# avi2924/Speech-Intent-Recognizer

Measured on AMD Instinct MI355X. Metric: utterances/sec (16 kHz, 3 s clips), inference: HIP STFT+mel+CNN/BiGRU forward + argmax, higher is better.
Workload: dtype f32

## Files before the change

speech-intent-recognizer_amd/csrc/f16x3_kernels.h:

```cpp
#pragma once
#include "bf16x6_kernels.h"

constexpr int H3_BM = 160, H3_BN = 256, H3_BK = 32;
constexpr int H3_APLANE = H3_BM * 64, H3_BPLANE = H3_BN * 64;
constexpr int H3_BOFF = 2 * H3_APLANE;
constexpr int H3_STAGE = H3_BOFF + 2 * H3_BPLANE;
constexpr int H3_APIECES = 2 * H3_BM / 16, H3_PIECES = H3_APIECES + 2 * H3_BN / 16;
constexpr int H3_PPW = (H3_PIECES + 7) / 8;
constexpr int h3_lds_bytes(int nst) { return nst * H3_STAGE; }

template <int BM>
struct H3Geo {
    static_assert(BM == 96 || BM == 128 || BM == 160, "BM = 96, 128 or 160");
    static constexpr int FR = BM / 32, ARG = BM / 16;
    static constexpr int APLANE = BM * 64, BOFF = 2 * APLANE, STAGE = BOFF + 2 * H3_BPLANE;
    static constexpr int APIECES = 2 * ARG, PIECES = APIECES + 2 * H3_BN / 16;
    static constexpr int PPW = (PIECES + 7) / 8, PREM = PIECES & 7;
    static constexpr int ISTRIDE = 3 * FR / PPW;
};
static_assert(H3Geo<H3_BM>::STAGE == H3_STAGE && H3Geo<H3_BM>::PIECES == H3_PIECES && H3Geo<H3_BM>::PPW == H3_PPW, "160-row geometry");

template <int FR>
__device__ __forceinline__ void h3_read_step(unsigned aaddr, unsigned baddr, f16x8 (&ah)[FR], f16x8 (&al)[FR], f16x8& bh, f16x8& bl) {
    if constexpr (FR == 5) {
        asm volatile(
            "ds_read_b128 %0, %12\n\t"
            "ds_read_b128 %10, %13 offset:20480\n\t"
            "ds_read_b128 %5, %12 offset:10240\n\t"
            "ds_read_b128 %11, %13 offset:36864\n\t"
            "ds_read_b128 %1, %12 offset:2048\n\t"
            "ds_read_b128 %6, %12 offset:12288\n\t"
            "ds_read_b128 %2, %12 offset:4096\n\t"
            "ds_read_b128 %7, %12 offset:14336\n\t"
            "ds_read_b128 %3, %12 offset:6144\n\t"
            "ds_read_b128 %8, %12 offset:16384\n\t"
            "ds_read_b128 %4, %12 offset:8192\n\t"
            "ds_read_b128 %9, %12 offset:18432\n\t"
            "s_waitcnt lgkmcnt(0)"
            : "=&v"(ah[0]), "=&v"(ah[1]), "=&v"(ah[2]), "=&v"(ah[3]), "=&v"(ah[4]),
              "=&v"(al[0]), "=&v"(al[1]), "=&v"(al[2]), "=&v"(al[3]), "=&v"(al[4]), "=&v"(bh), "=&v"(bl)
            : "v"(aaddr), "v"(baddr)
            : "memory");
    } else if constexpr (FR == 4) {
        asm volatile(
            "ds_read_b128 %0, %10\n\t"
            "ds_read_b128 %8, %11 offset:16384\n\t"
            "ds_read_b128 %4, %10 offset:8192\n\t"
            "ds_read_b128 %9, %11 offset:32768\n\t"
            "ds_read_b128 %1, %10 offset:2048\n\t"
            "ds_read_b128 %5, %10 offset:10240\n\t"
            "ds_read_b128 %2, %10 offset:4096\n\t"
            "ds_read_b128 %6, %10 offset:12288\n\t"
            "ds_read_b128 %3, %10 offset:6144\n\t"
            "ds_read_b128 %7, %10 offset:14336\n\t"
            "s_waitcnt lgkmcnt(0)"
            : "=&v"(ah[0]), "=&v"(ah[1]), "=&v"(ah[2]), "=&v"(ah[3]),
              "=&v"(al[0]), "=&v"(al[1]), "=&v"(al[2]), "=&v"(al[3]), "=&v"(bh), "=&v"(bl)
            : "v"(aaddr), "v"(baddr)
            : "memory");
    } else {
        static_assert(FR == 3, "3, 4 or 5 fragments");
        asm volatile(
            "ds_read_b128 %0, %8\n\t"
            "ds_read_b128 %6, %9 offset:12288\n\t"
            "ds_read_b128 %3, %8 offset:6144\n\t"
            "ds_read_b128 %7, %9 offset:28672\n\t"
            "ds_read_b128 %1, %8 offset:2048\n\t"
            "ds_read_b128 %4, %8 offset:8192\n\t"
            "ds_read_b128 %2, %8 offset:4096\n\t"
            "ds_read_b128 %5, %8 offset:10240\n\t"
            "s_waitcnt lgkmcnt(0)"
            : "=&v"(ah[0]), "=&v"(ah[1]), "=&v"(ah[2]), "=&v"(al[0]), "=&v"(al[1]), "=&v"(al[2]), "=&v"(bh), "=&v"(bl)
            : "v"(aaddr), "v"(baddr)
            : "memory");
    }
}

template <int NST, int KNOCK, int BM, bool GATHER>
__device__ __forceinline__ void h3_gemm_tile(
    const unsigned short* __restrict__ Ap, const unsigned short* __restrict__ Bp0, const unsigned short* __restrict__ Bp1,
    const float* __restrict__ bias0, const float* __restrict__ bias1, float* __restrict__ C, int ldc, int M, int MA, int N, int K,
    int wgid, const int* __restrict__ rows, int* rtab) {
    static_assert(NST == 2 || NST == 3, "two or three stages");
    using G = H3Geo<BM>;
    constexpr int FR = G::FR, PPW = G::PPW;
    extern __shared__ __attribute__((aligned(1024))) unsigned char h3_smem[];
    const int nbd = N / H3_BN, nb = 2 * nbd;
    const int mblk = wgid / nb, nbk = wgid - mblk * nb, z = nbk / nbd;
    const int m0 = mblk * BM, n0 = (nbk - z * nbd) * H3_BN;
    const unsigned short* __restrict__ Bp = z ? Bp1 : Bp0;
    const float* __restrict__ bias = z ? bias1 : bias0;
    const int tid = threadIdx.x, lane = tid & 63, wv = __builtin_amdgcn_readfirstlane(tid >> 6), m = lane & 31, h = lane >> 5;
    const size_t planeA = (size_t)MA * K, planeB = (size_t)N * K;

    const int lr = lane >> 2;
    const int csrc = (lane & 3) ^ ((lr >> 2) & 3);
    constexpr int AI = (G::APIECES + 7) / 8;
    int arow[AI];
#pragma unroll
    for (int i = 0; i < AI; ++i) {
        const int g = wv + 8 * i < G::APIECES ? wv + 8 * i : 0;
        const int row = m0 + (g % G::ARG) * 16 + lr;
        arow[i] = row < M ? row : M - 1;
    }
    int orow = 0;
    if (GATHER) {
        const int ro = m0 + tid < M ? m0 + tid : M - 1;
        orow = rows[ro];
#pragma unroll
        for (int i = 0; i < AI; ++i) arow[i] = rows[arow[i]];
    }
    unsigned int poff[PPW];
#pragma unroll
    for (int i = 0; i < PPW; ++i) {
        const int g = wv + 8 * i;
        const int gb = g - G::APIECES, pl = (gb >> 4) & 1, rg = gb & 15;
        if (GATHER) {
            const unsigned pa = i < AI ? (unsigned)((g < G::APIECES ? g / G::ARG : 0) * planeA + (size_t)arow[i < AI ? i : 0] * K + csrc * 8) : 0u;
            const unsigned pb = (unsigned)(pl * planeB + (size_t)(n0 + rg * 16 + lr) * K + csrc * 8);
            poff[i] = g < G::APIECES ? pa : pb;
        } else if (g < G::APIECES) {
            poff[i] = (unsigned int)(g / G::ARG * planeA + (size_t)arow[i < AI ? i : 0] * K + csrc * 8);
        } else {
            poff[i] = (unsigned int)(pl * planeB + (size_t)(n0 + rg * 16 + lr) * K + csrc * 8);
        }
    }
    if (GATHER) rtab[tid] = orow;
    auto piece = [&](int i, int kt, int buf) {
        if (KNOCK & 1) return;
        const int g = wv + 8 * i;
        if (g < G::PIECES) {
            const unsigned short* src = (g < G::APIECES ? Ap : Bp) + poff[i] + (size_t)kt * H3_BK;
            __builtin_amdgcn_global_load_lds((sir_gptr_t)src, (sir_lptr_t)(h3_smem + buf * G::STAGE + g * 1024), 16, 0, 0);
        }
    };

    f32x16 acc0[FR], acc1[FR];
#pragma unroll
    for (int mt = 0; mt < FR; ++mt)
#pragma unroll
        for (int r = 0; r < 16; ++r) { acc0[mt][r] = 0.0f; acc1[mt][r] = 0.0f; }

    const unsigned sbase = (unsigned)(uintptr_t)h3_smem;
    unsigned fa[2], fb[2];
#pragma unroll
    for (int ks = 0; ks < 2; ++ks) {
        fa[ks] = sbase + m * 64 + ((((ks << 1) | h) ^ ((m >> 2) & 3)) << 4);
        fb[ks] = fa[ks] + wv * 2048;
    }
    const int nk = K / H3_BK;

    auto compute = [&](int buf, auto issue_c, int ktn, int bufn) {
        constexpr bool ISSUE = decltype(issue_c)::value;
        const unsigned so = (unsigned)(buf * G::STAGE);
#pragma unroll
        for (int ks = 0; ks < 2; ++ks) {
            f16x8 ah[FR], al[FR], bh, bl;
            h3_read_step<FR>(fa[ks] + so, fb[ks] + so, ah, al, bh, bl);
#pragma unroll
            for (int t = 0; t < 3; ++t)
#pragma unroll
                for (int mt = 0; mt < FR; ++mt) {
                    if (KNOCK & 4) {
                        acc0[mt][0] += (float)ah[mt][0] * (float)bh[0] + (float)al[mt][1] * (float)bl[1];
                    } else {
                        if (t == 0) acc1[mt] = __builtin_amdgcn_mfma_f32_32x32x16_f16(al[mt], bh, acc1[mt], 0, 0, 0);
                        if (t == 1) acc1[mt] = __builtin_amdgcn_mfma_f32_32x32x16_f16(ah[mt], bl, acc1[mt], 0, 0, 0);
                        if (t == 2) acc0[mt] = __builtin_amdgcn_mfma_f32_32x32x16_f16(ah[mt], bh, acc0[mt], 0, 0, 0);
                    }
                    const int idx = t * FR + mt;
                    if (ISSUE && idx % G::ISTRIDE == G::ISTRIDE - 1 && idx / G::ISTRIDE < PPW && ks == (wv >> 2))
                        piece(idx / G::ISTRIDE, ktn, bufn);
                }
            __builtin_amdgcn_sched_barrier(0);
        }
    };

#pragma unroll
    for (int s = 0; s < NST - 1; ++s)
        if (s < nk) {
#pragma unroll
            for (int i = 0; i < PPW; ++i) piece(i, s, s);
        }
    auto tile_wait = [&](bool more) {
        if (NST == 2 || !more) asm volatile("s_waitcnt vmcnt(0)" ::: "memory");
        else if (G::PREM == 0 || wv < G::PREM) asm volatile("s_waitcnt vmcnt(%0)" :: "n"(PPW) : "memory");
        else asm volatile("s_waitcnt vmcnt(%0)" :: "n"(PPW - 1) : "memory");
        asm volatile("s_barrier" ::: "memory");
    };
    int buf = 0, bufn = NST - 1, kt = 0;
    for (; kt + NST - 1 < nk; ++kt) {
        tile_wait(true);
        compute(buf, std::true_type{}, kt + NST - 1, bufn);
        buf = buf + 1 == NST ? 0 : buf + 1;
        bufn = bufn + 1 == NST ? 0 : bufn + 1;
    }
    for (; kt < nk; ++kt) {
        tile_wait(kt + 1 < nk);
        compute(buf, std::false_type{}, 0, 0);
        buf = buf + 1 == NST ? 0 : buf + 1;
    }

    const int n = n0 + wv * 32 + m;
    const float bv = bias ? bias[n] : 0.0f;
    if (GATHER) {
        float* cz = C + (size_t)z * N + n;
#pragma unroll
        for (int mt = 0; mt < FR; ++mt)
#pragma unroll
            for (int i = 0; i < 4; ++i) {
                const int4 g4 = *reinterpret_cast<const int4*>(rtab + mt * 32 + 8 * i + 4 * h);
                const int gr[4] = {g4.x, g4.y, g4.z, g4.w};
#pragma unroll
                for (int j = 0; j < 4; ++j) cz[gr[j] * ldc] = fmaf(acc1[mt][4 * i + j], H3_LO_INV, acc0[mt][4 * i + j]) + bv;
            }
        return;
    }
    float* crow = C + (size_t)(m0 + 4 * h) * ldc + (size_t)z * N + n;
    if (m0 + BM <= M) {
#pragma unroll
        for (int mt = 0; mt < FR; ++mt)
#pragma unroll
            for (int r = 0; r < 16; ++r)
                crow[(size_t)(mt * 32 + (r & 3) + 8 * (r >> 2)) * ldc] = fmaf(acc1[mt][r], H3_LO_INV, acc0[mt][r]) + bv;
    } else {
#pragma unroll
        for (int mt = 0; mt < FR; ++mt)
#pragma unroll
            for (int r = 0; r < 16; ++r) {
                const int ro = mt * 32 + (r & 3) + 8 * (r >> 2);
                if (m0 + 4 * h + ro < M) crow[(size_t)ro * ldc] = fmaf(acc1[mt][r], H3_LO_INV, acc0[mt][r]) + bv;
            }
    }
}

__device__ __forceinline__ int h3_xcd_tile(int orig, int nt) {
    const int xcd = orig & 7, q = nt >> 3, rem = nt & 7;
    return (xcd < rem ? xcd * (q + 1) : rem * (q + 1) + (xcd - rem) * q) + (orig >> 3);
}

template <int NST = 3, int KNOCK = 0>
static __global__ __launch_bounds__(512) void gemm_nt_f16x3_kernel(
    const unsigned short* __restrict__ Ap, const unsigned short* __restrict__ Bp0, const unsigned short* __restrict__ Bp1,
    const float* __restrict__ bias0, const float* __restrict__ bias1, float* __restrict__ C, int ldc, int M, int N, int K) {
    h3_gemm_tile<NST, KNOCK, H3_BM, false>(Ap, Bp0, Bp1, bias0, bias1, C, ldc, M, M, N, K, h3_xcd_tile(blockIdx.x, gridDim.x), nullptr, nullptr);
}

__host__ __device__ constexpr int h3_gather_tiles(int bm, int count, int N) { return (count + bm - 1) / bm * 2 * (N / H3_BN); }
__host__ __device__ constexpr int h3_gather_bm(int count, int N, int ncu) {
    return h3_gather_tiles(96, count, N) <= ncu ? 96 : h3_gather_tiles(128, count, N) <= ncu ? 128 : 160;
}
__host__ __device__ constexpr int h3_gather_cost(int bm, int K) {
    return K > 512 ? (bm == 96 ? 402 : bm == 128 ? 447 : 513) : (bm == 96 ? 236 : bm == 128 ? 261 : 294);
}
constexpr int H3_TP_FLOOR = 108;
__host__ __device__ constexpr int h3_gather_bm_throughput(int count, int N, int K, int ncu) {
    if (h3_gather_tiles(96, count, N) <= H3_TP_FLOOR) return h3_gather_bm(count, N, ncu);
    const int c96 = (count + 95) / 96 * h3_gather_cost(96, K), c128 = (count + 127) / 128 * h3_gather_cost(128, K),
              c160 = (count + 159) / 160 * h3_gather_cost(160, K);
    return c96 <= c128 && c96 <= c160 ? 96 : c128 <= c160 ? 128 : 160;
}

template <int KNOCK = 0, int FBM = 0>
static __global__ __launch_bounds__(512) void gemm_nt_f16x3_gather_kernel(
    const unsigned short* __restrict__ Ap, const unsigned short* __restrict__ Bp0, const unsigned short* __restrict__ Bp1,
    const float* __restrict__ bias0, const float* __restrict__ bias1, float* __restrict__ C, int ldc, const int* __restrict__ rows,
    int MA, int N, int K, int ncu, int throughput, int* __restrict__ rec) {
    __shared__ __attribute__((aligned(16))) int rtab[512];
    const int count = rows[0];
    const int bm = FBM ? FBM : throughput ? h3_gather_bm_throughput(count, N, K, ncu) : h3_gather_bm(count, N, ncu);
    const int nt = h3_gather_tiles(bm, count, N);
    if (blockIdx.x == 0 && threadIdx.x == 0 && rec) { rec[0] = count; rec[1] = bm; }
    if ((int)blockIdx.x >= nt) return;
    const int wgid = h3_xcd_tile(blockIdx.x, nt);
    if (bm == 96) h3_gemm_tile<3, KNOCK, 96, true>(Ap, Bp0, Bp1, bias0, bias1, C, ldc, count, MA, N, K, wgid, rows + 1, rtab);
    else if (bm == 128) h3_gemm_tile<3, KNOCK, 128, true>(Ap, Bp0, Bp1, bias0, bias1, C, ldc, count, MA, N, K, wgid, rows + 1, rtab);
    else if (count < MA) h3_gemm_tile<3, KNOCK, 160, true>(Ap, Bp0, Bp1, bias0, bias1, C, ldc, count, MA, N, K, wgid, rows + 1, rtab);
    else h3_gemm_tile<3, KNOCK, 160, false>(Ap, Bp0, Bp1, bias0, bias1, C, ldc, MA, MA, N, K, wgid, nullptr, nullptr);
}

static inline bool gemm_f16x3_ok(int M, int N, int K) {
    return N % H3_BN == 0 && K % H3_BK == 0 && (size_t)2 * M * K < ((size_t)1 << 31) && (size_t)2 * N * K < ((size_t)1 << 31);
}

static inline int launch_gemm_nt_f16x3(sir_handle* h, hipStream_t st, const unsigned short* Ap, const unsigned short* Bp0,
                                              const unsigned short* Bp1, const float* bias0, const float* bias1, float* C, int ldc,
                                              int M, int N, int K) {
    SIR_HIP_TRY(gemm_f16x3_ok(M, N, K) ? hipSuccess : hipErrorInvalidValue);
    SIR_TRY(sir_lds_opt_in(h, (const void*)gemm_nt_f16x3_kernel<3, 0>, h3_lds_bytes(3)));
    const int nwg = ((M + H3_BM - 1) / H3_BM) * 2 * (N / H3_BN);
    hipLaunchKernelGGL((gemm_nt_f16x3_kernel<3, 0>), dim3(nwg), dim3(512), h3_lds_bytes(3), st, Ap, Bp0, Bp1, bias0, bias1, C, ldc, M, N, K);
    SIR_KCHECK();
    return SIR_OK;
}

static inline int launch_gemm_nt_f16x3_gather(sir_handle* h, hipStream_t st, const unsigned short* Ap, const unsigned short* Bp0,
                                                     const unsigned short* Bp1, const float* bias0, const float* bias1, float* C, int ldc,
                                                     const int* rows, int MA, int N, int K, bool throughput, int* rec) {
    SIR_HIP_TRY(gemm_f16x3_ok(MA, N, K) && K >= 2 * H3_BK && (size_t)MA * ldc < ((size_t)1 << 31) ? hipSuccess : hipErrorInvalidValue);
    SIR_TRY(sir_lds_opt_in(h, (const void*)gemm_nt_f16x3_gather_kernel<0, 0>, h3_lds_bytes(3)));
    hipLaunchKernelGGL((gemm_nt_f16x3_gather_kernel<0, 0>), dim3(h3_gather_tiles(96, MA, N)), dim3(512), h3_lds_bytes(3), st, Ap, Bp0, Bp1,
                       bias0, bias1, C, ldc, rows, MA, N, K, h->num_cus, throughput ? 1 : 0, rec);
    SIR_KCHECK();
    return SIR_OK;
}
```

Before: 787,100.

## Overlap LDS fragment reads with MFMAs via per-fragment lgkmcnt waits

Replaces the block LDS read with a full lgkmcnt(0) wait by individually issued ds_read_b128 loads. Graduated waits let each MFMA start as soon as its own fragment arrives, and the second k-step's fragments are prefetched while the first k-step's MFMAs run. The gather tile-size cost table is retuned to match, and an optional s_memtime debug-stamp path is added behind a template flag. The change costs more live VGPRs for the double set of fragments and depends on the order in which lgkmcnt counts down.

```diff
diff --git a/speech-intent-recognizer_amd/csrc/f16x3_kernels.h b/speech-intent-recognizer_amd/csrc/f16x3_kernels.h
--- a/speech-intent-recognizer_amd/csrc/f16x3_kernels.h
+++ b/speech-intent-recognizer_amd/csrc/f16x3_kernels.h
@@ -20,63 +20,58 @@
 };
 static_assert(H3Geo<H3_BM>::STAGE == H3_STAGE && H3Geo<H3_BM>::PIECES == H3_PIECES && H3Geo<H3_BM>::PPW == H3_PPW, "160-row geometry");
 
-template <int FR>
-__device__ __forceinline__ void h3_read_step(unsigned aaddr, unsigned baddr, f16x8 (&ah)[FR], f16x8 (&al)[FR], f16x8& bh, f16x8& bl) {
-    if constexpr (FR == 5) {
-        asm volatile(
-            "ds_read_b128 %0, %12\n\t"
-            "ds_read_b128 %10, %13 offset:20480\n\t"
-            "ds_read_b128 %5, %12 offset:10240\n\t"
-            "ds_read_b128 %11, %13 offset:36864\n\t"
-            "ds_read_b128 %1, %12 offset:2048\n\t"
-            "ds_read_b128 %6, %12 offset:12288\n\t"
-            "ds_read_b128 %2, %12 offset:4096\n\t"
-            "ds_read_b128 %7, %12 offset:14336\n\t"
-            "ds_read_b128 %3, %12 offset:6144\n\t"
-            "ds_read_b128 %8, %12 offset:16384\n\t"
-            "ds_read_b128 %4, %12 offset:8192\n\t"
-            "ds_read_b128 %9, %12 offset:18432\n\t"
-            "s_waitcnt lgkmcnt(0)"
-            : "=&v"(ah[0]), "=&v"(ah[1]), "=&v"(ah[2]), "=&v"(ah[3]), "=&v"(ah[4]),
-              "=&v"(al[0]), "=&v"(al[1]), "=&v"(al[2]), "=&v"(al[3]), "=&v"(al[4]), "=&v"(bh), "=&v"(bl)
-            : "v"(aaddr), "v"(baddr)
-            : "memory");
-    } else if constexpr (FR == 4) {
-        asm volatile(
-            "ds_read_b128 %0, %10\n\t"
-            "ds_read_b128 %8, %11 offset:16384\n\t"
-            "ds_read_b128 %4, %10 offset:8192\n\t"
-            "ds_read_b128 %9, %11 offset:32768\n\t"
-            "ds_read_b128 %1, %10 offset:2048\n\t"
-            "ds_read_b128 %5, %10 offset:10240\n\t"
-            "ds_read_b128 %2, %10 offset:4096\n\t"
-            "ds_read_b128 %6, %10 offset:12288\n\t"
-            "ds_read_b128 %3, %10 offset:6144\n\t"
-            "ds_read_b128 %7, %10 offset:14336\n\t"
-            "s_waitcnt lgkmcnt(0)"
-            : "=&v"(ah[0]), "=&v"(ah[1]), "=&v"(ah[2]), "=&v"(ah[3]),
-              "=&v"(al[0]), "=&v"(al[1]), "=&v"(al[2]), "=&v"(al[3]), "=&v"(bh), "=&v"(bl)
-            : "v"(aaddr), "v"(baddr)
-            : "memory");
-    } else {
-        static_assert(FR == 3, "3, 4 or 5 fragments");
-        asm volatile(
-            "ds_read_b128 %0, %8\n\t"
-            "ds_read_b128 %6, %9 offset:12288\n\t"
-            "ds_read_b128 %3, %8 offset:6144\n\t"
-            "ds_read_b128 %7, %9 offset:28672\n\t"
-            "ds_read_b128 %1, %8 offset:2048\n\t"
-            "ds_read_b128 %4, %8 offset:8192\n\t"
-            "ds_read_b128 %2, %8 offset:4096\n\t"
-            "ds_read_b128 %5, %8 offset:10240\n\t"
-            "s_waitcnt lgkmcnt(0)"
-            : "=&v"(ah[0]), "=&v"(ah[1]), "=&v"(ah[2]), "=&v"(al[0]), "=&v"(al[1]), "=&v"(al[2]), "=&v"(bh), "=&v"(bl)
-            : "v"(aaddr), "v"(baddr)
-            : "memory");
-    }
-}
-
-template <int NST, int KNOCK, int BM, bool GATHER>
+template <int OFF>
+__device__ __forceinline__ void h3_read(f16x8& d, unsigned addr) {
+    asm volatile("ds_read_b128 %0, %1 offset:%2" : "=v"(d) : "v"(addr), "n"(OFF) : "memory");
+}
+template <int BM>
+__device__ __forceinline__ void h3_issue_step(unsigned aaddr, unsigned baddr, f16x8 (&ah)[BM / 32], f16x8 (&al)[BM / 32], f16x8& bh, f16x8& bl) {
+    using G = H3Geo<BM>;
+    h3_read<G::BOFF>(bh, baddr);
+    h3_read<G::APLANE>(al[0], aaddr);
+    if constexpr (G::FR > 1) h3_read<G::APLANE + 2048>(al[1], aaddr);
+    if constexpr (G::FR > 2) h3_read<G::APLANE + 4096>(al[2], aaddr);
+    if constexpr (G::FR > 3) h3_read<G::APLANE + 6144>(al[3], aaddr);
+    if constexpr (G::FR > 4) h3_read<G::APLANE + 8192>(al[4], aaddr);
+    h3_read<G::BOFF + H3_BPLANE>(bl, baddr);
+    h3_read<0>(ah[0], aaddr);
+    if constexpr (G::FR > 1) h3_read<2048>(ah[1], aaddr);
+    if constexpr (G::FR > 2) h3_read<4096>(ah[2], aaddr);
+    if constexpr (G::FR > 3) h3_read<6144>(ah[3], aaddr);
+    if constexpr (G::FR > 4) h3_read<8192>(ah[4], aaddr);
+}
+template <int BM, int OFF>
+__device__ __forceinline__ void h3_issue_a(unsigned aaddr, f16x8 (&a)[BM / 32]) {
+    h3_read<OFF>(a[0], aaddr);
+    h3_read<OFF + 2048>(a[1], aaddr);
+    h3_read<OFF + 4096>(a[2], aaddr);
+    if constexpr (BM > 96) h3_read<OFF + 6144>(a[3], aaddr);
+    if constexpr (BM > 128) h3_read<OFF + 8192>(a[4], aaddr);
+}
+template <int N>
+__device__ __forceinline__ void h3_wait(f16x8& a) { asm volatile("s_waitcnt lgkmcnt(%1)" : "+v"(a) : "n"(N)); }
+template <int N>
+__device__ __forceinline__ void h3_wait(f16x8& a, f16x8& b) { asm volatile("s_waitcnt lgkmcnt(%2)" : "+v"(a), "+v"(b) : "n"(N)); }
+template <int N0, int FR>
+__device__ __forceinline__ void h3_wait_frag(int mt, f16x8& b, f16x8 (&a)[FR]) {
+    if (mt == 0) h3_wait<N0>(b, a[0]);
+    if (mt == 1) h3_wait<N0 - 1>(a[1]);
+    if (mt == 2) h3_wait<N0 - 2>(a[2]);
+    if constexpr (FR > 3) { if (mt == 3) h3_wait<N0 - 3>(a[3]); }
+    if constexpr (FR > 4) { if (mt == 4) h3_wait<N0 - 4>(a[4]); }
+}
+
+constexpr int H3_DBG_T0 = 4, H3_DBG_NT = 6;
+__device__ unsigned h3_dbg_stamps[64];
+__device__ __forceinline__ unsigned h3_stamp(unsigned acc, int slot) {
+    unsigned long long t;
+    __builtin_amdgcn_sched_barrier(0);
+    asm volatile("s_memtime %0\n\ts_waitcnt lgkmcnt(0)" : "=s"(t) :: "memory");
+    __builtin_amdgcn_sched_barrier(0);
+    return (int)(threadIdx.x & 63) == slot ? (unsigned)t : acc;
+}
+
+template <int NST, int KNOCK, int BM, bool GATHER, int DBG = 0>
 __device__ __forceinline__ void h3_gemm_tile(
     const unsigned short* __restrict__ Ap, const unsigned short* __restrict__ Bp0, const unsigned short* __restrict__ Bp1,
     const float* __restrict__ bias0, const float* __restrict__ bias1, float* __restrict__ C, int ldc, int M, int MA, int N, int K,
@@ -150,29 +145,74 @@
     }
     const int nk = K / H3_BK;
 
-    auto compute = [&](int buf, auto issue_c, int ktn, int bufn) {
+    const bool dbg_on = (DBG & 1) && blockIdx.x == 0 && wv == 0;
+    unsigned stamps = 0;
+    auto stamp = [&](int ds, int slot) {
+        if (DBG & 1) { if (dbg_on && ds >= 0) stamps = h3_stamp(stamps, ds + slot); }
+    };
+
+    auto row = [&](auto t_c, auto n0_c, auto issue_c, int ks, f16x8 (&ah)[FR], f16x8 (&al)[FR], f16x8& bh, f16x8& bl, int ktn, int bufn, int ds) {
+        constexpr int T = decltype(t_c)::value, N0 = decltype(n0_c)::value;
         constexpr bool ISSUE = decltype(issue_c)::value;
+#pragma unroll
+        for (int mt = 0; mt < FR; ++mt) {
+            if constexpr (N0 >= 0 && T == 0) h3_wait_frag<N0, FR>(mt, bh, al);
+            if constexpr (N0 >= 0 && T == 1) h3_wait_frag<N0, FR>(mt, bl, ah);
+            if (!(DBG & 2) && T == 1 && mt == FR - 1) stamp(ds, 3 + 4 * ks);
+            if (KNOCK & 4) {
+                if (T == 2) acc0[mt][0] += (float)ah[mt][0] * (float)bh[0] + (float)al[mt][1] * (float)bl[1];
+            } else {
+                if (T == 0) acc1[mt] = __builtin_amdgcn_mfma_f32_32x32x16_f16(al[mt], bh, acc1[mt], 0, 0, 0);
+                if (T == 1) acc1[mt] = __builtin_amdgcn_mfma_f32_32x32x16_f16(ah[mt], bl, acc1[mt], 0, 0, 0);
+                if (T == 2) acc0[mt] = __builtin_amdgcn_mfma_f32_32x32x16_f16(ah[mt], bh, acc0[mt], 0, 0, 0);
+            }
+            const int idx = T * FR + mt;
+            if (ISSUE && idx % G::ISTRIDE == G::ISTRIDE - 1 && idx / G::ISTRIDE < PPW && ks == (wv >> 2)) {
+                piece(idx / G::ISTRIDE, ktn, bufn);
+                if (idx / G::ISTRIDE == PPW - 1) stamp(ds, 4 + 4 * ks);
+            }
+        }
+        if (T == 2) stamp(ds, 5 + 4 * ks);
+        __builtin_amdgcn_sched_barrier(0);
+    };
+    using I0 = std::integral_constant<int, 0>; using I1 = std::integral_constant<int, 1>; using I2 = std::integral_constant<int, 2>;
+    using NOWAIT = std::integral_constant<int, -1>;
+    constexpr int NRD = 2 * FR + 2;
+
+    auto compute = [&](int buf, auto issue_c, int ktn, int bufn, int ds) {
         const unsigned so = (unsigned)(buf * G::STAGE);
-#pragma unroll
-        for (int ks = 0; ks < 2; ++ks) {
-            f16x8 ah[FR], al[FR], bh, bl;
-            h3_read_step<FR>(fa[ks] + so, fb[ks] + so, ah, al, bh, bl);
-#pragma unroll
-            for (int t = 0; t < 3; ++t)
-#pragma unroll
-                for (int mt = 0; mt < FR; ++mt) {
-                    if (KNOCK & 4) {
-                        acc0[mt][0] += (float)ah[mt][0] * (float)bh[0] + (float)al[mt][1] * (float)bl[1];
-                    } else {
-                        if (t == 0) acc1[mt] = __builtin_amdgcn_mfma_f32_32x32x16_f16(al[mt], bh, acc1[mt], 0, 0, 0);
-                        if (t == 1) acc1[mt] = __builtin_amdgcn_mfma_f32_32x32x16_f16(ah[mt], bl, acc1[mt], 0, 0, 0);
-                        if (t == 2) acc0[mt] = __builtin_amdgcn_mfma_f32_32x32x16_f16(ah[mt], bh, acc0[mt], 0, 0, 0);
-                    }
-                    const int idx = t * FR + mt;
-                    if (ISSUE && idx % G::ISTRIDE == G::ISTRIDE - 1 && idx / G::ISTRIDE < PPW && ks == (wv >> 2))
-                        piece(idx / G::ISTRIDE, ktn, bufn);
+        if constexpr ((DBG & 6) != 0) {
+#pragma unroll
+            for (int ks = 0; ks < 2; ++ks) {
+                f16x8 ah[FR], al[FR], bh, bl;
+                h3_issue_step<BM>(fa[ks] + so, fb[ks] + so, ah, al, bh, bl);
+                if constexpr ((DBG & 2) != 0) {
+                    stamp(ds, 2 + 4 * ks);
+                    asm volatile("s_waitcnt lgkmcnt(0)" ::: "memory");
+                    __builtin_amdgcn_sched_barrier(0);
+                    stamp(ds, 3 + 4 * ks);
                 }
-            __builtin_amdgcn_sched_barrier(0);
+                row(I0{}, std::integral_constant<int, NRD - 2>{}, issue_c, ks, ah, al, bh, bl, ktn, bufn, ds);
+                row(I1{}, std::integral_constant<int, FR - 1>{}, issue_c, ks, ah, al, bh, bl, ktn, bufn, ds);
+                row(I2{}, NOWAIT{}, issue_c, ks, ah, al, bh, bl, ktn, bufn, ds);
+            }
+        } else {
+            f16x8 ah[FR], al[FR], bh, bl, ah1[FR], al1[FR], bh1, bl1;
+            const unsigned a0 = fa[0] + so, b0 = fb[0] + so, a1 = fa[1] + so, b1 = fb[1] + so;
+            h3_issue_step<BM>(a0, b0, ah, al, bh, bl);
+            row(I0{}, std::integral_constant<int, NRD - 2>{}, issue_c, 0, ah, al, bh, bl, ktn, bufn, ds);
+            h3_issue_a<BM, H3Geo<BM>::APLANE>(a1, al1);
+            row(I1{}, std::integral_constant<int, 2 * FR - 1>{}, issue_c, 0, ah, al, bh, bl, ktn, bufn, ds);
+            h3_read<G::BOFF>(bh1, b1);
+            row(I2{}, NOWAIT{}, issue_c, 0, ah, al, bh, bl, ktn, bufn, ds);
+            h3_read<G::BOFF + H3_BPLANE>(bl1, b1);
+            h3_issue_a<BM, 0>(a1, ah1);
+            h3_wait<FR + 1>(bh1, al1[0]);
+#pragma unroll
+            for (int mt = 1; mt < FR; ++mt) h3_wait<FR + 1>(al1[mt]);
+            row(I0{}, NOWAIT{}, issue_c, 1, ah1, al1, bh1, bl1, ktn, bufn, ds);
+            row(I1{}, std::integral_constant<int, FR - 1>{}, issue_c, 1, ah1, al1, bh1, bl1, ktn, bufn, ds);
+            row(I2{}, NOWAIT{}, issue_c, 1, ah1, al1, bh1, bl1, ktn, bufn, ds);
         }
     };
 
@@ -182,25 +222,34 @@
 #pragma unroll
             for (int i = 0; i < PPW; ++i) piece(i, s, s);
         }
-    auto tile_wait = [&](bool more) {
+    auto tile_wait = [&](bool more, int ds) {
         if (NST == 2 || !more) asm volatile("s_waitcnt vmcnt(0)" ::: "memory");
         else if (G::PREM == 0 || wv < G::PREM) asm volatile("s_waitcnt vmcnt(%0)" :: "n"(PPW) : "memory");
         else asm volatile("s_waitcnt vmcnt(%0)" :: "n"(PPW - 1) : "memory");
+        stamp(ds, 0);
         asm volatile("s_barrier" ::: "memory");
+        stamp(ds, 1);
+    };
+    auto dbg_slot = [&](int kt) {
+        if ((DBG & 1) && kt == H3_DBG_T0) stamp(0, 60);
+        return (DBG & 1) && kt >= H3_DBG_T0 && kt < H3_DBG_T0 + H3_DBG_NT ? 10 * (kt - H3_DBG_T0) : -1;
     };
     int buf = 0, bufn = NST - 1, kt = 0;
     for (; kt + NST - 1 < nk; ++kt) {
-        tile_wait(true);
-        compute(buf, std::true_type{}, kt + NST - 1, bufn);
+        const int ds = dbg_slot(kt);
+        tile_wait(true, ds);
+        compute(buf, std::true_type{}, kt + NST - 1, bufn, ds);
         buf = buf + 1 == NST ? 0 : buf + 1;
         bufn = bufn + 1 == NST ? 0 : bufn + 1;
     }
     for (; kt < nk; ++kt) {
-        tile_wait(kt + 1 < nk);
-        compute(buf, std::false_type{}, 0, 0);
+        const int ds = dbg_slot(kt);
+        tile_wait(kt + 1 < nk, ds);
+        compute(buf, std::false_type{}, 0, 0, ds);
         buf = buf + 1 == NST ? 0 : buf + 1;
     }
 
+    if ((DBG & 1) && dbg_on) h3_dbg_stamps[lane] = stamps;
     const int n = n0 + wv * 32 + m;
     const float bv = bias ? bias[n] : 0.0f;
     if (GATHER) {
@@ -251,7 +300,7 @@
     return h3_gather_tiles(96, count, N) <= ncu ? 96 : h3_gather_tiles(128, count, N) <= ncu ? 128 : 160;
 }
 __host__ __device__ constexpr int h3_gather_cost(int bm, int K) {
-    return K > 512 ? (bm == 96 ? 402 : bm == 128 ? 447 : 513) : (bm == 96 ? 236 : bm == 128 ? 261 : 294);
+    return K > 512 ? (bm == 96 ? 392 : bm == 128 ? 434 : 487) : (bm == 96 ? 226 : bm == 128 ? 248 : 283);
 }
 constexpr int H3_TP_FLOOR = 108;
 __host__ __device__ constexpr int h3_gather_bm_throughput(int count, int N, int K, int ncu) {
@@ -261,7 +310,7 @@
     return c96 <= c128 && c96 <= c160 ? 96 : c128 <= c160 ? 128 : 160;
 }
 
-template <int KNOCK = 0, int FBM = 0>
+template <int KNOCK = 0, int FBM = 0, int DBG = 0>
 static __global__ __launch_bounds__(512) void gemm_nt_f16x3_gather_kernel(
     const unsigned short* __restrict__ Ap, const unsigned short* __restrict__ Bp0, const unsigned short* __restrict__ Bp1,
     const float* __restrict__ bias0, const float* __restrict__ bias1, float* __restrict__ C, int ldc, const int* __restrict__ rows,
@@ -273,10 +322,10 @@
     if (blockIdx.x == 0 && threadIdx.x == 0 && rec) { rec[0] = count; rec[1] = bm; }
     if ((int)blockIdx.x >= nt) return;
     const int wgid = h3_xcd_tile(blockIdx.x, nt);
-    if (bm == 96) h3_gemm_tile<3, KNOCK, 96, true>(Ap, Bp0, Bp1, bias0, bias1, C, ldc, count, MA, N, K, wgid, rows + 1, rtab);
-    else if (bm == 128) h3_gemm_tile<3, KNOCK, 128, true>(Ap, Bp0, Bp1, bias0, bias1, C, ldc, count, MA, N, K, wgid, rows + 1, rtab);
-    else if (count < MA) h3_gemm_tile<3, KNOCK, 160, true>(Ap, Bp0, Bp1, bias0, bias1, C, ldc, count, MA, N, K, wgid, rows + 1, rtab);
-    else h3_gemm_tile<3, KNOCK, 160, false>(Ap, Bp0, Bp1, bias0, bias1, C, ldc, MA, MA, N, K, wgid, nullptr, nullptr);
+    if (bm == 96) h3_gemm_tile<3, KNOCK, 96, true, DBG>(Ap, Bp0, Bp1, bias0, bias1, C, ldc, count, MA, N, K, wgid, rows + 1, rtab);
+    else if (bm == 128) h3_gemm_tile<3, KNOCK, 128, true, DBG>(Ap, Bp0, Bp1, bias0, bias1, C, ldc, count, MA, N, K, wgid, rows + 1, rtab);
+    else if (count < MA) h3_gemm_tile<3, KNOCK, 160, true, DBG>(Ap, Bp0, Bp1, bias0, bias1, C, ldc, count, MA, N, K, wgid, rows + 1, rtab);
+    else h3_gemm_tile<3, KNOCK, 160, false, DBG>(Ap, Bp0, Bp1, bias0, bias1, C, ldc, MA, MA, N, K, wgid, nullptr, nullptr);
 }
 
 static inline bool gemm_f16x3_ok(int M, int N, int K) {
```

After: 779,500 (median of 2 runs). Within noise of the previous version (-1.0%).
